# megvii-research/CVPR2023-UniDistill

Hardware: AMD Instinct MI355X
Metric: distill-train samples/sec (nuScenes frame); bev_pool+voxelize HBM GB/s (higher is better)
Workload: dtype f32; 1 GPU; camera_exp_distill_lidar: student+teacher distillation step, 6 cams 256x704, 30000-pt cloud, 40 GT boxes, fwd+bwd+AdamW; batch_per_gpu=4, global_batch=4, parallelism=dp1, layout=channels-last dense convs, executor=eager+DDP, strict_no_library_fallthrough=True, wgrad_stream=on, ranks=1, dist_backend=none (single process)

## Files before the change

### cvpr2023-unidistill_amd/csrc/bn_act.hip

```cpp
#include "ud_common.h"
#include "ud_prof.h"
#include "ud_reduce.h"

namespace {

constexpr int kMaxSlices = 1024;
int group_width(int C) { return C % 64 == 0 ? 64 : (C % 32 == 0 ? 32 : 16); }
int slices_for(long long P, int C) {
  const int gw = group_width(C), groups = C / gw;
  long long s = 2048 / (groups > 0 ? groups : 1);
  const long long cap = (P + 256 / (gw / 8) - 1) / (256 / (gw / 8));
  if (s > cap) s = cap;
  if (s < 1) s = 1;
  if (s > kMaxSlices) s = kMaxSlices;
  return (int)s;
}

__device__ __forceinline__ float bf_lo(unsigned u) { return __uint_as_float(u << 16); }
__device__ __forceinline__ float bf_hi(unsigned u) { return __uint_as_float(u & 0xFFFF0000u); }

__device__ __forceinline__ void unpack8(const uint4& r, float* v) {
  v[0] = bf_lo(r.x); v[1] = bf_hi(r.x); v[2] = bf_lo(r.y); v[3] = bf_hi(r.y);
  v[4] = bf_lo(r.z); v[5] = bf_hi(r.z); v[6] = bf_lo(r.w); v[7] = bf_hi(r.w);
}
__device__ __forceinline__ uint4 pack8(const float* v) {
  return make_uint4(ud_pack_bf16x2(v[0], v[1]), ud_pack_bf16x2(v[2], v[3]),
                    ud_pack_bf16x2(v[4], v[5]), ud_pack_bf16x2(v[6], v[7]));
}
__device__ __forceinline__ void ld8(const unsigned short* p, float* v) { unpack8(*reinterpret_cast<const uint4*>(p), v); }
__device__ __forceinline__ void st8(unsigned short* p, const float* v) { *reinterpret_cast<uint4*>(p) = pack8(v); }
__device__ __forceinline__ void ld8(const float* p, float* v) {
  const float4 a = *reinterpret_cast<const float4*>(p), b = *reinterpret_cast<const float4*>(p + 4);
  v[0] = a.x; v[1] = a.y; v[2] = a.z; v[3] = a.w; v[4] = b.x; v[5] = b.y; v[6] = b.z; v[7] = b.w;
}
__device__ __forceinline__ void st8(float* p, const float* v) {
  *reinterpret_cast<float4*>(p) = make_float4(v[0], v[1], v[2], v[3]);
  *reinterpret_cast<float4*>(p + 4) = make_float4(v[4], v[5], v[6], v[7]);
}
__device__ __forceinline__ float elem_f(unsigned short u) { return __uint_as_float((unsigned)u << 16); }
__device__ __forceinline__ float elem_f(float u) { return u; }

__device__ __forceinline__ void load8(const float* p, float* v) {
  const float4 a = *reinterpret_cast<const float4*>(p), b = *reinterpret_cast<const float4*>(p + 4);
  v[0] = a.x; v[1] = a.y; v[2] = a.z; v[3] = a.w; v[4] = b.x; v[5] = b.y; v[6] = b.z; v[7] = b.w;
}

template <typename T>
__global__ __launch_bounds__(256) void k_bn_act_fwd(const T* __restrict__ x, const T* __restrict__ res,
                                                    const float* __restrict__ scale,
                                                    const float* __restrict__ shift, T* __restrict__ y,
                                                    long long P, int C, int CH, int relu, long long y_ld) {
  const int chunk = blockIdx.y * CH + threadIdx.x % CH, lanes = 256 / CH, pl = threadIdx.x / CH;
  if (chunk * 8 >= C) return;
  float s[8], t[8];
  load8(scale + chunk * 8, s);
  load8(shift + chunk * 8, t);
  for (long long p = (long long)blockIdx.x * lanes + pl; p < P; p += (long long)gridDim.x * lanes) {
    const size_t off = (size_t)p * C + chunk * 8;
    float v[8];
    ld8(x + off, v);
#pragma unroll
    for (int e = 0; e < 8; ++e) v[e] = fmaf(v[e], s[e], t[e]);
    if (res) {
      float r[8];
      ld8(res + off, r);
#pragma unroll
      for (int e = 0; e < 8; ++e) v[e] += r[e];
    }
    if (relu) {
#pragma unroll
      for (int e = 0; e < 8; ++e) v[e] = fmaxf(v[e], 0.f);
    }
    st8(y + (size_t)p * y_ld + chunk * 8, v);
  }
}

__device__ __forceinline__ void masked_grad(const float* xv, const float* yv, bool has_y, const float* dyv,
                                            const float* s, const float* t, int relu, float* dr) {
  if (!relu) {
#pragma unroll
    for (int e = 0; e < 8; ++e) dr[e] = dyv[e];
    return;
  }
  if (has_y) {
#pragma unroll
    for (int e = 0; e < 8; ++e) dr[e] = yv[e] > 0.f ? dyv[e] : 0.f;
  } else {
#pragma unroll
    for (int e = 0; e < 8; ++e) dr[e] = fmaf(xv[e], s[e], t[e]) > 0.f ? dyv[e] : 0.f;
  }
}

template <int GW>
struct GroupMap {
  static constexpr int kChunks = GW / 8, kLanes = 256 / kChunks;
};

template <int GW, typename T>
__global__ __launch_bounds__(256) void k_bn_stats_partial(const T* __restrict__ x, long long P,
                                                          int C, float* __restrict__ partial) {
  using M = GroupMap<GW>;
  __shared__ float red[M::kLanes][GW + 1][2];
  const int cg = blockIdx.y, tid = threadIdx.x, chunk = tid % M::kChunks, pl = tid / M::kChunks;
  const int c0 = cg * GW + chunk * 8;
  float piv[8], s1[8], s2[8];
  ld8(x + c0, piv);
#pragma unroll
  for (int e = 0; e < 8; ++e) s1[e] = s2[e] = 0.f;
  for (long long p = (long long)blockIdx.x * M::kLanes + pl; p < P; p += (long long)gridDim.x * M::kLanes) {
    float v[8];
    ld8(x + (size_t)p * C + c0, v);
#pragma unroll
    for (int e = 0; e < 8; ++e) {
      const float d = v[e] - piv[e];
      s1[e] += d;
      s2[e] += d * d;
    }
  }
#pragma unroll
  for (int e = 0; e < 8; ++e) { red[pl][chunk * 8 + e][0] = s1[e]; red[pl][chunk * 8 + e][1] = s2[e]; }
  __syncthreads();
  if (tid < 2 * GW) {
    const int c = tid >> 1, w = tid & 1;
    float a = 0.f;
    for (int i = 0; i < M::kLanes; ++i) a += red[i][c][w];
    partial[((size_t)blockIdx.x * C + cg * GW + c) * 2 + w] = a;
  }
}

template <typename T>
__global__ __launch_bounds__(256) void k_bn_stats_final(const T* __restrict__ x, const float* __restrict__ partial,
                                 int slices, long long P, int C, const float* __restrict__ gamma,
                                 const float* __restrict__ beta, float eps, float* __restrict__ mean,
                                 float* __restrict__ var, float* __restrict__ invstd,
                                 float* __restrict__ scale, float* __restrict__ shift,
                                 float* __restrict__ running_mean, float* __restrict__ running_var,
                                 float momentum, long long* __restrict__ batches_tracked) {
  __shared__ double red[16][16][2];
  const int tid = threadIdx.x, cl = tid & 15, sl = tid >> 4;
  const int c = blockIdx.x * 16 + cl;
  if (batches_tracked && blockIdx.x == 0 && tid == 0) *batches_tracked += 1;
  auto ld = [&](int s) { return *reinterpret_cast<const float2*>(partial + ((size_t)s * C + c) * 2); };
  double a0 = 0.0, a1 = 0.0, a2 = 0.0, a3 = 0.0, q0 = 0.0, q1 = 0.0, q2 = 0.0, q3 = 0.0;
  int s = sl;
  for (; s + 48 < slices; s += 64) {
    const float2 v0 = ld(s), v1 = ld(s + 16), v2 = ld(s + 32), v3 = ld(s + 48);
    a0 += v0.x; q0 += v0.y;
    a1 += v1.x; q1 += v1.y;
    a2 += v2.x; q2 += v2.y;
    a3 += v3.x; q3 += v3.y;
  }
  for (; s < slices; s += 16) {
    const float2 v = ld(s);
    a0 += v.x; q0 += v.y;
  }
  double a = (a0 + a1) + (a2 + a3), q = (q0 + q1) + (q2 + q3);
  red[sl][cl][0] = a;
  red[sl][cl][1] = q;
  __syncthreads();
  if (sl != 0) return;
  a = q = 0.0;
  for (int k = 0; k < 16; ++k) {
    a += red[k][cl][0];
    q += red[k][cl][1];
  }
  const double piv = x ? (double)elem_f(x[c]) : 0.0;
  const double m = a / (double)P;
  double v = q / (double)P - m * m;
  if (v < 0.0) v = 0.0;
  const float mu = (float)(piv + m), is = (float)(1.0 / sqrt(v + (double)eps));
  mean[c] = mu;
  var[c] = (float)v;
  invstd[c] = is;
  const float sc = gamma[c] * is;
  scale[c] = sc;
  shift[c] = beta[c] - mu * sc;
  if (running_mean) {
    const double unbiased = v * ((double)P / (double)(P > 1 ? P - 1 : 1));
    running_mean[c] = (1.f - momentum) * running_mean[c] + momentum * mu;
    running_var[c] = (1.f - momentum) * running_var[c] + momentum * (float)unbiased;
  }
}

template <int GW, typename T>
__global__ __launch_bounds__(256) void k_bn_bwd_reduce(const T* __restrict__ x, const T* __restrict__ y,
                                                       const T* __restrict__ dy,
                                                       const float* __restrict__ scale,
                                                       const float* __restrict__ shift,
                                                       const float* __restrict__ mean, long long P,
                                                       int C, int relu, float* __restrict__ partial, long long dy_ld) {
  using M = GroupMap<GW>;
  __shared__ float red[M::kLanes][GW + 1][2];
  const int cg = blockIdx.y, tid = threadIdx.x, chunk = tid % M::kChunks, pl = tid / M::kChunks;
  const int c0 = cg * GW + chunk * 8;
  float s[8], t[8], mu[8], s1[8], s2[8];
  load8(scale + c0, s);
  load8(shift + c0, t);
  load8(mean + c0, mu);
#pragma unroll
  for (int e = 0; e < 8; ++e) s1[e] = s2[e] = 0.f;
  for (long long p = (long long)blockIdx.x * M::kLanes + pl; p < P; p += (long long)gridDim.x * M::kLanes) {
    const size_t off = (size_t)p * C + c0;
    float xv[8], dyv[8], dr[8], yv[8];
    ld8(x + off, xv);
    ld8(dy + (size_t)p * dy_ld + c0, dyv);
    if (y) ld8(y + off, yv);
    masked_grad(xv, yv, y != nullptr, dyv, s, t, relu, dr);
#pragma unroll
    for (int e = 0; e < 8; ++e) {
      s1[e] += dr[e];
      s2[e] += dr[e] * (xv[e] - mu[e]);
    }
  }
// ... 168 lines not shown
      a1 += elem_f(xp[(size_t)(p + step) * ld]);
    }
    if (p < P) a0 += elem_f(xp[(size_t)p * ld]);
  }
  red[tid] = a0 + a1;
  __syncthreads();
  if (tid < cw) {
    float a = 0.f;
    for (int i = 0; i < R; ++i) a += red[i * cw + tid];
    partial[(size_t)blockIdx.x * C + cb0 + tid] = a;
  }
}

struct BnWs { float *partial, *k0, *k2; };
size_t carve(UdArena& ar, int C, BnWs* w) {
  w->partial = ar.take<float>((size_t)kMaxSlices * C * 2);
  w->k0 = ar.take<float>(C);
  w->k2 = ar.take<float>(C);
  return ar.used;
}
void stream_grid(long long P, int C, int* CH, dim3* grid) {
  const int chunks = C / 8;
  int ch = 1;
  while (ch < chunks && ch < 256) ch <<= 1;
  const int lanes = 256 / ch, cblocks = (chunks + ch - 1) / ch;
  long long slices = (P + lanes - 1) / lanes;
  const long long want = 4096 / cblocks > 0 ? 4096 / cblocks : 1;
  if (slices > want) slices = want;
  if (slices < 1) slices = 1;
  *CH = ch;
  *grid = dim3((unsigned)slices, (unsigned)cblocks);
}

}

template <typename T>
int bn_stats_impl(const T* x, long long P, int C, const float* gamma, const float* beta, float eps,
                  float* mean, float* var, float* invstd, float* scale, float* shift, float* running_mean,
                  float* running_var, float momentum, long long* batches_tracked, void* workspace,
                  size_t workspace_bytes, hipStream_t stream) {
  if (!x || !gamma || !beta || !mean || !var || !invstd || !scale || !shift || P <= 0 || C <= 0 ||
      ((running_mean == nullptr) != (running_var == nullptr)))
    return UD_ERR_INVALID_ARG;
  if (C % 16) return UD_ERR_UNSUPPORTED;
  UdArena ar(workspace, workspace_bytes);
  BnWs w;
  carve(ar, C, &w);
  if (!ar.ok()) return UD_ERR_WORKSPACE;
  UdProfScope prof("bn_act.stats", stream);
  const int slices = slices_for(P, C), gw = group_width(C);
  if (gw == 64)
    k_bn_stats_partial<64, T><<<dim3(slices, C / 64), 256, 0, stream>>>(x, P, C, w.partial);
  else if (gw == 32)
    k_bn_stats_partial<32, T><<<dim3(slices, C / 32), 256, 0, stream>>>(x, P, C, w.partial);
  else
    k_bn_stats_partial<16, T><<<dim3(slices, C / 16), 256, 0, stream>>>(x, P, C, w.partial);
  UD_LAUNCH_CHECK();
  k_bn_stats_final<T><<<C / 16, 256, 0, stream>>>(x, w.partial, slices, P, C, gamma, beta, eps, mean, var, invstd, scale,
                                            shift, running_mean, running_var, momentum, batches_tracked);
  UD_LAUNCH_CHECK();
  return UD_OK;
}

template <typename T>
int bn_fwd_impl(const T* x, const T* residual, const float* scale, const float* shift, T* y, long long P, int C,
                int relu, long long y_ld, hipStream_t stream) {
// ... 140 lines not shown
                              float* shift, float* running_mean, float* running_var, float momentum,
                              long long* batches_tracked, ud_stream_t stream) {
  if (!partial || slices <= 0 || !gamma || !beta || !mean || !var || !invstd || !scale || !shift || P <= 0 || C <= 0 ||
      ((running_mean == nullptr) != (running_var == nullptr)))
    return UD_ERR_INVALID_ARG;
  UdProfScope prof("bn_act.stats", (hipStream_t)stream);
  if (C % 16) return UD_ERR_UNSUPPORTED;
  k_bn_stats_final<float><<<C / 16, 256, 0, (hipStream_t)stream>>>(nullptr, partial, slices, P, C, gamma, beta, eps, mean, var,
                                                              invstd, scale, shift, running_mean, running_var, momentum,
                                                              batches_tracked);
  UD_LAUNCH_CHECK();
  return UD_OK;
}

int ud_bn_act_fwd(const void* x, const void* residual, const float* scale, const float* shift, void* y,
                  long long P, int C, int relu, ud_stream_t stream) {
  return bn_fwd_impl<bf16_t>((const bf16_t*)x, (const bf16_t*)residual, scale, shift, (bf16_t*)y, P, C, relu, C,
                             (hipStream_t)stream);
}
int ud_bn_act_fwd_f32(const float* x, const float* residual, const float* scale, const float* shift, float* y,
                      long long P, int C, int relu, ud_stream_t stream) {
  return bn_fwd_impl<float>(x, residual, scale, shift, y, P, C, relu, C, (hipStream_t)stream);
}
int ud_bn_act_fwd_ld(const void* x, const void* residual, const float* scale, const float* shift, void* y,
                     long long P, int C, long long y_ld, int relu, ud_stream_t stream) {
  return bn_fwd_impl<bf16_t>((const bf16_t*)x, (const bf16_t*)residual, scale, shift, (bf16_t*)y, P, C, relu, y_ld,
                             (hipStream_t)stream);
}
int ud_bn_act_fwd_ld_f32(const float* x, const float* residual, const float* scale, const float* shift, float* y,
                         long long P, int C, long long y_ld, int relu, ud_stream_t stream) {
  return bn_fwd_impl<float>(x, residual, scale, shift, y, P, C, relu, y_ld, (hipStream_t)stream);
}

int ud_bn_act_bwd(const void* x, const void* y, const void* dy, const float* scale, const float* shift,
                  const float* mean, const float* invstd, void* dx, void* dresidual, float* dgamma,
                  float* dbeta, long long P, int C, int relu, void* workspace, size_t workspace_bytes,
                  ud_stream_t stream) {
  return bn_bwd_impl<bf16_t>((const bf16_t*)x, (const bf16_t*)y, (const bf16_t*)dy, scale, shift, mean, invstd,
                             (bf16_t*)dx, (bf16_t*)dresidual, dgamma, dbeta, P, C, relu, C, workspace, workspace_bytes,
                             (hipStream_t)stream);
}
int ud_bn_act_bwd_f32(const float* x, const float* y, const float* dy, const float* scale, const float* shift,
                      const float* mean, const float* invstd, float* dx, float* dresidual, float* dgamma,
                      float* dbeta, long long P, int C, int relu, void* workspace, size_t workspace_bytes,
                      ud_stream_t stream) {
  return bn_bwd_impl<float>(x, y, dy, scale, shift, mean, invstd, dx, dresidual, dgamma, dbeta, P, C, relu, C, workspace,
                            workspace_bytes, (hipStream_t)stream);
}
int ud_bn_act_bwd_ld(const void* x, const void* y, const void* dy, long long dy_ld, const float* scale, const float* shift,
                     const float* mean, const float* invstd, void* dx, void* dresidual, float* dgamma,
                     float* dbeta, long long P, int C, int relu, void* workspace, size_t workspace_bytes,
                     ud_stream_t stream) {
  return bn_bwd_impl<bf16_t>((const bf16_t*)x, (const bf16_t*)y, (const bf16_t*)dy, scale, shift, mean, invstd,
                             (bf16_t*)dx, (bf16_t*)dresidual, dgamma, dbeta, P, C, relu, dy_ld, workspace, workspace_bytes,
                             (hipStream_t)stream);
}
int ud_bn_act_bwd_ld_f32(const float* x, const float* y, const float* dy, long long dy_ld, const float* scale,
                         const float* shift, const float* mean, const float* invstd, float* dx, float* dresidual,
                         float* dgamma, float* dbeta, long long P, int C, int relu, void* workspace,
                         size_t workspace_bytes, ud_stream_t stream) {
  return bn_bwd_impl<float>(x, y, dy, scale, shift, mean, invstd, dx, dresidual, dgamma, dbeta, P, C, relu, dy_ld,
                            workspace, workspace_bytes, (hipStream_t)stream);
}
int ud_bn_act_bwd_frozen_ld(const void* x, const void* y, const void* dy, long long dy_ld, const float* scale,
                            const float* shift, const float* mean, const float* invstd, void* dx, void* dresidual,
                            float* dgamma, float* dbeta, long long P, int C, int relu, void* workspace,
// ... 25 lines not shown
```

### cvpr2023-unidistill_amd/csrc/ud_reduce.h

```cpp
#ifndef UD_REDUCE_H_
#define UD_REDUCE_H_
#include "ud_common.h"

namespace {

__global__ __launch_bounds__(256) void k_wgrad_sum(const float* __restrict__ partial, int slices, size_t n,
                                                   float* __restrict__ out) {
  __shared__ float4 part[4][64];
  const int lane = threadIdx.x & 63, wave = threadIdx.x >> 6;
  const size_t i4 = (size_t)blockIdx.x * 64 + lane, n4 = n / 4;
  float4 a = make_float4(0.f, 0.f, 0.f, 0.f);
  if (i4 < n4) {
    const int per = (slices + 3) / 4, s0 = wave * per, s1 = min(slices, s0 + per);
    auto ld = [&](int s) { return *reinterpret_cast<const float4*>(partial + (size_t)s * n + 4 * i4); };
    int s = s0;
    for (; s + 3 < s1; s += 4) {
      const float4 v0 = ld(s), v1 = ld(s + 1), v2 = ld(s + 2), v3 = ld(s + 3);
      a.x += v0.x; a.y += v0.y; a.z += v0.z; a.w += v0.w;
      a.x += v1.x; a.y += v1.y; a.z += v1.z; a.w += v1.w;
      a.x += v2.x; a.y += v2.y; a.z += v2.z; a.w += v2.w;
      a.x += v3.x; a.y += v3.y; a.z += v3.z; a.w += v3.w;
    }
    for (; s < s1; ++s) {
      const float4 v = ld(s);
// ... 57 lines not shown
#pragma unroll
  for (int o = 32; o > 0; o >>= 1) {
    a += __shfl_xor(a, o);
    q += __shfl_xor(q, o);
  }
  if (T > 64) {
    if (lane == 0) { red[wv][0] = a; red[wv][1] = q; }
    __syncthreads();
    if (tid == 0) {
      a = red[0][0], q = red[0][1];
#pragma unroll
      for (int w = 1; w < T / 64; ++w) { a += red[w][0]; q += red[w][1]; }
    }
  }
  if (tid != 0) return;
  const float is = invstd[c], dg = q * is, inv_p = 1.0f / (float)P;
  dbeta[c] = a;
  dgamma[c] = dg;
  const float kk2 = -scale[c] * (dg * inv_p) * is;
  k2[c] = kk2;
  k0[c] = -scale[c] * (a * inv_p) - kk2 * mean[c];
}

inline int ud_bn_bwd_final(const float* partial, int slices, int C, long long P, const float* scale, const float* mean,
                           const float* invstd, float* dgamma, float* dbeta, float* k0, float* k2, hipStream_t stream) {
  if (slices > 128)
    k_bn_bwd_final<256><<<C, 256, 0, stream>>>(partial, slices, C, P, scale, mean, invstd, dgamma, dbeta, k0, k2);
  else
    k_bn_bwd_final<64><<<C, 64, 0, stream>>>(partial, slices, C, P, scale, mean, invstd, dgamma, dbeta, k0, k2);
  UD_LAUNCH_CHECK();
  return UD_OK;
}

template <int T, typename V>
__device__ __forceinline__ V ud_colsum_block(const V* __restrict__ partial, int slices, int C, int c, V* __restrict__ red) {
  const int tid = threadIdx.x, lane = tid & 63, wv = tid >> 6;
  V a0 = 0, a1 = 0, a2 = 0, a3 = 0;
  int s = tid;
  for (; s + 3 * T < slices; s += 4 * T) {
    const V v0 = partial[(size_t)s * C + c], v1 = partial[(size_t)(s + T) * C + c], v2 = partial[(size_t)(s + 2 * T) * C + c],
            v3 = partial[(size_t)(s + 3 * T) * C + c];
    a0 += v0; a1 += v1; a2 += v2; a3 += v3;
  }
  for (; s < slices; s += T) a0 += partial[(size_t)s * C + c];
  V a = (a0 + a1) + (a2 + a3);
#pragma unroll
  for (int o = 32; o > 0; o >>= 1) a += __shfl_xor(a, o);
  if (T > 64) {
    if (lane == 0) red[wv] = a;
    __syncthreads();
    if (tid == 0) {
      a = red[0];
#pragma unroll
      for (int w = 1; w < T / 64; ++w) a += red[w];
    }
  }
  return a;
}

template <int T>
__global__ __launch_bounds__(T) void k_colsum_final(const float* __restrict__ partial, int slices, int C, float* __restrict__ out) {
  __shared__ float red[T / 64];
  const float a = ud_colsum_block<T, float>(partial, slices, C, blockIdx.x, red);
  if (threadIdx.x == 0) out[blockIdx.x] = a;
}

// ... 56 lines not shown
```

### cvpr2023-unidistill_amd/unidistill_amd/ops/bn_act.py

```python
import torch

from .. import _lib


def supported(x, bn):
    if not (x.is_cuda and x.dtype in (torch.bfloat16, torch.float32) and x.dim() in (2, 4) and x.shape[1] % 16 == 0
            and x.shape[0] > 0 and bn.affine and bn.track_running_stats and bn.momentum is not None):
        return False
    return x.is_contiguous() if x.dim() == 2 else x.is_contiguous(memory_format=torch.channels_last)


def _like(t, ref):
    t = t.to(ref.dtype)
    return t.contiguous() if ref.dim() == 2 else t.contiguous(memory_format=torch.channels_last)


def _row_stride(t, ref):
    if t.dim() != 4 or ref.dim() != 4 or t.dtype != ref.dtype or t.shape != ref.shape or not t.is_cuda:
        return None
    B, C, H, W = t.shape
    s = t.stride()
    ld = s[3] if W > 1 else (s[2] if H > 1 else C)
    if ld < C or ld % 8 or t.data_ptr() % 16 or (C > 1 and s[1] != 1) or (W > 1 and s[3] != ld) or (H > 1 and s[2] != W * ld) \
            or (B > 1 and s[0] != H * W * ld):
        return None
    return ld


_ws_bytes = {}


def _workspace(dev, C):
    n = _ws_bytes.get(C)
    if n is None:
        n = _ws_bytes[C] = _lib.load().ud_bn_act_workspace_bytes(C)
    return _lib.workspace(dev, n, "bn_act")


def batch_stats(x, gamma, beta, running_mean, running_var, training, momentum, eps, tracked=None, partial=None):
    _lib.require_gpu(x, gamma, beta)
    f32 = x.dtype == torch.float32
    k_stats = _lib.ud.ud_bn_stats_f32 if f32 else _lib.ud.ud_bn_stats
    C = x.shape[1]
    P = x.numel() // C
    dev = x.device
    g32 = gamma.detach() if gamma.dtype == torch.float32 else gamma.detach().float()
    b32 = beta.detach() if beta.dtype == torch.float32 else beta.detach().float()
    stream = _lib.stream_of(x)
    if training:
        vec = torch.empty((5, C), dtype=torch.float32, device=dev)
        v0, row = vec.data_ptr(), 4 * C
        ws = _workspace(dev, C)
        fp32_buffers = running_mean is not None and running_mean.dtype == torch.float32
        rm, rv = (running_mean, running_var) if fp32_buffers else (None, None)
        if partial is not None and partial[2] == P:
            _lib.ud.ud_bn_stats_from_partials(partial[0].data_ptr(), int(partial[1]), P, C, g32.data_ptr(), b32.data_ptr(),
                                              float(eps), v0, v0 + row, v0 + 2 * row, v0 + 3 * row, v0 + 4 * row, rm, rv,
                                              float(momentum or 0.0), tracked, stream)
        else:
            k_stats(x.data_ptr(), P, C, g32.data_ptr(), b32.data_ptr(), float(eps), v0, v0 + row, v0 + 2 * row, v0 + 3 * row,
                    v0 + 4 * row, rm, rv, float(momentum or 0.0), tracked, ws.data_ptr(), ws.numel(), stream)
        if rm is not None:
            torch.autograd.graph.increment_version(rm)
            torch.autograd.graph.increment_version(rv)
        if running_mean is not None and not fp32_buffers:
            with torch.no_grad():
                running_mean.mul_(1 - momentum).add_(vec[0], alpha=momentum)
                running_var.mul_(1 - momentum).add_(vec[1], alpha=momentum * P / max(P - 1, 1))
        return vec
    def fold():
        invstd = torch.rsqrt(running_var.float() + eps)
        mean = running_mean.float()
        scale = g32 * invstd
        return torch.stack((mean, invstd * invstd, invstd, scale, b32 - mean * scale))

    if gamma.requires_grad or beta.requires_grad or torch.cuda.is_current_stream_capturing():
        if getattr(running_var, "_ud_bn_eval", None) is not None and not torch.cuda.is_current_stream_capturing():
            running_var._ud_bn_eval = None
        return fold()
    key = (running_mean._version, running_var._version, gamma._version, beta._version, float(eps),
           running_mean.data_ptr(), running_var.data_ptr(), gamma.data_ptr(), beta.data_ptr())
    hit = getattr(running_var, "_ud_bn_eval", None)
    if hit is not None and hit[0] == key:
        return hit[1]
    vec = fold()
    try:
        running_var._ud_bn_eval = (key, vec)
    except (AttributeError, RuntimeError):
# ... 10 lines not shown


def drop_colsum(g):
    if getattr(g, "_ud_colsum", None) is not None:
        g._ud_colsum = None


def bias_grad(gy):
    hit = getattr(gy, "_ud_colsum", None)
    if hit is not None and hit[0] == gy._version and hit[1] == gy.data_ptr():
        return hit[2]
    C = gy.shape[1]
    rows = gy.dim() == 2 and gy.is_contiguous()
    maps = gy.dim() == 4 and gy.is_contiguous(memory_format=torch.channels_last)
    if not (gy.is_cuda and gy.dtype in (torch.float32, torch.bfloat16) and (rows or maps) and gy.numel() > 0):
        dims = (0,) if gy.dim() == 2 else (0, 2, 3)
        return gy.sum(dims, dtype=torch.float32)
    lib = _lib.load()
    out = torch.empty(C, dtype=torch.float32, device=gy.device)
    ws = _lib.workspace(gy.device, lib.ud_colsum_workspace_bytes(C), "colsum")
    fn = _lib.ud.ud_colsum_f32 if gy.dtype == torch.float32 else _lib.ud.ud_colsum_bf16
    fn(gy.data_ptr(), gy.numel() // C, C, C, out.data_ptr(), ws.data_ptr(), ws.numel(), _lib.stream_of(gy))
    return out


class _BnActFn(torch.autograd.Function):
    @staticmethod
    def forward(ctx, x, gamma, beta, residual, running_mean, running_var, training, momentum, eps, relu,
                tracked=None, partial=None, out=None):
        k_fwd = _lib.ud.ud_bn_act_fwd_ld_f32 if x.dtype == torch.float32 else _lib.ud.ud_bn_act_fwd_ld
        C = x.shape[1]
        P = x.numel() // C
        stream = _lib.stream_of(x)
        vec = batch_stats(x, gamma, beta, running_mean, running_var, training, momentum, eps, tracked, partial)
        v0, row = vec.data_ptr(), 4 * C
        if residual is not None:
            residual = _like(residual, x)
        y = torch.empty_like(x) if out is None else out[0]
        ld = C if out is None else _row_stride(y, x)
        if ld is None:
            raise ValueError(f"bn_act: out {tuple(y.shape)} strides {tuple(y.stride())} is not a channel slice of a channels-last map")
        k_fwd(x.data_ptr(), residual, v0 + 3 * row, v0 + 4 * row, y.data_ptr(), P, C, ld, 1 if relu else 0, stream)
        ctx.cfg = (bool(training), bool(relu), residual is not None)
        ctx.save_for_backward(x, y if (residual is not None and relu) else None, vec)
        return y

    @staticmethod
    def backward(ctx, dy):
        x, y, vec = ctx.saved_tensors
        training, relu, has_res = ctx.cfg
        if y is not None and y.stride() != x.stride():
            y = _like(y, x)
        C = x.shape[1]
        P = x.numel() // C
        ld = _row_stride(dy, x)
        if ld is None:
            dy, ld = _like(dy, x), C
        dx = torch.empty_like(x)
        dres = torch.empty_like(x) if (has_res and ctx.needs_input_grad[3]) else None
        if dres is not None and not relu:
            dres = None
        v0, row = vec.data_ptr(), 4 * C
        if training:
            dgb = torch.empty((2, C), dtype=torch.float32, device=x.device)
            ws = _workspace(x.device, C)
            g0 = dgb.data_ptr()
            k_bwd = _lib.ud.ud_bn_act_bwd_ld_f32 if x.dtype == torch.float32 else _lib.ud.ud_bn_act_bwd_ld
            k_bwd(x.data_ptr(), y, dy.data_ptr(), ld, v0 + 3 * row, v0 + 4 * row, v0, v0 + 2 * row, dx.data_ptr(), dres, g0,
                  g0 + row, P, C, 1 if relu else 0, ws.data_ptr(), ws.numel(), _lib.stream_of(x))
            dgamma, dbeta = dgb[0], dgb[1]
        else:
            k_bwd = _lib.ud.ud_bn_act_bwd_frozen_ld_f32 if x.dtype == torch.float32 else _lib.ud.ud_bn_act_bwd_frozen_ld
            dgamma = dbeta = dgb = ws = None
            if ctx.needs_input_grad[1] or ctx.needs_input_grad[2]:
                dgb = torch.empty((2, C), dtype=torch.float32, device=x.device)
# ... 64 lines not shown
```

### include/unidistill_hip.h

```cpp
#ifndef UNIDISTILL_HIP_H
#define UNIDISTILL_HIP_H

#include <stddef.h>
#include <stdint.h>

#ifdef __cplusplus
extern "C" {
#endif

typedef void* ud_stream_t;

#define UD_OK 0
#define UD_ERR_INVALID_ARG (-1)
#define UD_ERR_WORKSPACE (-2)
#define UD_ERR_HIP (-3)
#define UD_ERR_UNSUPPORTED (-4)

const char* ud_version(void);
int ud_abi_version(void);
const char* ud_error_string(int code);

void ud_prof_enable(int on);
int ud_prof_read(const char* name, double* total_ms, int* calls, int reset);

// ... 373 lines not shown
size_t ud_bn_act_workspace_bytes(int C);
int ud_bn_stats(const void* x, long long P, int C, const float* gamma, const float* beta, float eps,
                float* mean, float* var, float* invstd, float* scale, float* shift, float* running_mean,
                float* running_var, float momentum, long long* batches_tracked, void* workspace,
                size_t workspace_bytes, ud_stream_t stream);
int ud_bn_act_fwd(const void* x, const void* residual, const float* scale, const float* shift, void* y,
                  long long P, int C, int relu, ud_stream_t stream);
int ud_bn_act_bwd(const void* x, const void* y, const void* dy, const float* scale, const float* shift,
                  const float* mean, const float* invstd, void* dx, void* dresidual, float* dgamma,
                  float* dbeta, long long P, int C, int relu, void* workspace, size_t workspace_bytes,
                  ud_stream_t stream);
int ud_bn_stats_from_partials(const float* partial, int slices, long long P, int C, const float* gamma,
                              const float* beta, float eps, float* mean, float* var, float* invstd, float* scale,
                              float* shift, float* running_mean, float* running_var, float momentum,
                              long long* batches_tracked, ud_stream_t stream);
int ud_bn_stats_f32(const float* x, long long P, int C, const float* gamma, const float* beta, float eps,
                    float* mean, float* var, float* invstd, float* scale, float* shift, float* running_mean,
                    float* running_var, float momentum, long long* batches_tracked, void* workspace,
                    size_t workspace_bytes, ud_stream_t stream);
int ud_bn_act_fwd_f32(const float* x, const float* residual, const float* scale, const float* shift, float* y,
                      long long P, int C, int relu, ud_stream_t stream);
int ud_bn_act_bwd_f32(const float* x, const float* y, const float* dy, const float* scale, const float* shift,
                      const float* mean, const float* invstd, float* dx, float* dresidual, float* dgamma,
                      float* dbeta, long long P, int C, int relu, void* workspace, size_t workspace_bytes,
                      ud_stream_t stream);
int ud_bn_act_fwd_ld(const void* x, const void* residual, const float* scale, const float* shift, void* y,
                     long long P, int C, long long y_ld, int relu, ud_stream_t stream);
int ud_bn_act_fwd_ld_f32(const float* x, const float* residual, const float* scale, const float* shift, float* y,
                         long long P, int C, long long y_ld, int relu, ud_stream_t stream);
int ud_bn_act_bwd_ld(const void* x, const void* y, const void* dy, long long dy_ld, const float* scale, const float* shift,
                     const float* mean, const float* invstd, void* dx, void* dresidual, float* dgamma,
                     float* dbeta, long long P, int C, int relu, void* workspace, size_t workspace_bytes,
                     ud_stream_t stream);
int ud_bn_act_bwd_ld_f32(const float* x, const float* y, const float* dy, long long dy_ld, const float* scale,
                         const float* shift, const float* mean, const float* invstd, float* dx, float* dresidual,
                         float* dgamma, float* dbeta, long long P, int C, int relu, void* workspace,
                         size_t workspace_bytes, ud_stream_t stream);
int ud_bn_act_bwd_frozen_ld(const void* x, const void* y, const void* dy, long long dy_ld, const float* scale,
                            const float* shift, const float* mean, const float* invstd, void* dx, void* dresidual,
                            float* dgamma, float* dbeta, long long P, int C, int relu, void* workspace,
                            size_t workspace_bytes, ud_stream_t stream);
int ud_bn_act_bwd_frozen_ld_f32(const float* x, const float* y, const float* dy, long long dy_ld, const float* scale,
                                const float* shift, const float* mean, const float* invstd, float* dx, float* dresidual,
                                float* dgamma, float* dbeta, long long P, int C, int relu, void* workspace,
                                size_t workspace_bytes, ud_stream_t stream);

size_t ud_nms_bev_workspace_bytes(int N);
int ud_nms_rotated_bev(const float* boxes, int N, float thresh, long long* keep, int* num_keep,
                       void* workspace, size_t workspace_bytes, ud_stream_t stream);
int ud_boxes_iou_bev(const float* a, int Na, const float* b, int Nb, float* iou, ud_stream_t stream);

size_t ud_proposal_workspace_bytes(int B, int T, int K);
int ud_proposal_layer(const float* const* heads, const long long* strides, const int* num_classes,
                      const int* class_offsets, const float* iou_alpha, int B, int T, int H, int W, int K,
                      int post_max, int box_dim, int no_log, float out_size_factor, float voxel_x,
                      float voxel_y, float pc_x, float pc_y, const float* center_range, float score_threshold,
                      float nms_threshold, float* rois, float* roi_scores, long long* roi_labels,
                      int* num_boxes, void* workspace, size_t workspace_bytes, ud_stream_t stream);

size_t ud_det_loss_workspace_bytes(int T);
int ud_det_focal_fwd(const float* const* hm, const long long* hm_bstride, const int* ncls, int T, int B,
                     int ncm, int HW, const float* gt, float alpha, float gamma, float* prob,
                     float* pos_neg, void* workspace, size_t workspace_bytes, ud_stream_t stream);
int ud_det_focal_bwd(const int* ncls, int T, int B, int ncm, int HW, const float* gt, const float* prob,
                     const float* g_prob, const float* g_pos, const float* g_neg, float alpha,
                     float gamma, float* dlogit, ud_stream_t stream);
// ... 284 lines not shown
```

Before: 70.06 samples/s.

## Fold BN stats finalization into the training forward apply kernel

Adds a training-mode BN forward path in which each apply block reduces the per-slice partial sums for its channel group, computes scale/shift in shared memory, and then applies BN+residual+ReLU. This removes the separate k_bn_stats_final launch and the global round-trip of scale/shift. The apply loop is also unrolled 4x to keep more loads in flight. In exchange, every block redundantly re-reduces the partials (only block 0 writes the stats), and the fold is limited to at most 64 slices, falling back to the old path otherwise.

```diff
diff --git a/cvpr2023-unidistill_amd/csrc/bn_act.hip b/cvpr2023-unidistill_amd/csrc/bn_act.hip
--- a/cvpr2023-unidistill_amd/csrc/bn_act.hip
+++ b/cvpr2023-unidistill_amd/csrc/bn_act.hip
@@ -43,6 +43,19 @@
 __device__ __forceinline__ void load8(const float* p, float* v) {
   const float4 a = *reinterpret_cast<const float4*>(p), b = *reinterpret_cast<const float4*>(p + 4);
   v[0] = a.x; v[1] = a.y; v[2] = a.z; v[3] = a.w; v[4] = b.x; v[5] = b.y; v[6] = b.z; v[7] = b.w;
+}
+
+__device__ __forceinline__ void bn_apply8(float* v, const float* r, bool has_r, const float* s, const float* t, int relu) {
+#pragma unroll
+  for (int e = 0; e < 8; ++e) v[e] = fmaf(v[e], s[e], t[e]);
+  if (has_r) {
+#pragma unroll
+    for (int e = 0; e < 8; ++e) v[e] += r[e];
+  }
+  if (relu) {
+#pragma unroll
+    for (int e = 0; e < 8; ++e) v[e] = fmaxf(v[e], 0.f);
+  }
 }
 
 template <typename T>
@@ -57,20 +70,10 @@
   load8(shift + chunk * 8, t);
   for (long long p = (long long)blockIdx.x * lanes + pl; p < P; p += (long long)gridDim.x * lanes) {
     const size_t off = (size_t)p * C + chunk * 8;
-    float v[8];
+    float v[8], r[8];
     ld8(x + off, v);
-#pragma unroll
-    for (int e = 0; e < 8; ++e) v[e] = fmaf(v[e], s[e], t[e]);
-    if (res) {
-      float r[8];
-      ld8(res + off, r);
-#pragma unroll
-      for (int e = 0; e < 8; ++e) v[e] += r[e];
-    }
-    if (relu) {
-#pragma unroll
-      for (int e = 0; e < 8; ++e) v[e] = fmaxf(v[e], 0.f);
-    }
+    if (res) ld8(res + off, r);
+    bn_apply8(v, r, res != nullptr, s, t, relu);
     st8(y + (size_t)p * y_ld + chunk * 8, v);
   }
 }
@@ -125,6 +128,21 @@
     float a = 0.f;
     for (int i = 0; i < M::kLanes; ++i) a += red[i][c][w];
     partial[((size_t)blockIdx.x * C + cg * GW + c) * 2 + w] = a;
+  }
+}
+
+__device__ __forceinline__ void bn_store_stats(const UdBnFwdStats& st, int c, float* __restrict__ mean, float* __restrict__ var,
+                                               float* __restrict__ invstd, float* __restrict__ scale, float* __restrict__ shift,
+                                               float* __restrict__ running_mean, float* __restrict__ running_var,
+                                               float momentum) {
+  mean[c] = st.mean;
+  var[c] = st.var;
+  invstd[c] = st.invstd;
+  scale[c] = st.scale;
+  shift[c] = st.shift;
+  if (running_mean) {
+    running_mean[c] = (1.f - momentum) * running_mean[c] + momentum * st.mean;
+    running_var[c] = (1.f - momentum) * running_var[c] + momentum * st.unbiased;
   }
 }
 
@@ -140,21 +158,8 @@
   const int tid = threadIdx.x, cl = tid & 15, sl = tid >> 4;
   const int c = blockIdx.x * 16 + cl;
   if (batches_tracked && blockIdx.x == 0 && tid == 0) *batches_tracked += 1;
-  auto ld = [&](int s) { return *reinterpret_cast<const float2*>(partial + ((size_t)s * C + c) * 2); };
-  double a0 = 0.0, a1 = 0.0, a2 = 0.0, a3 = 0.0, q0 = 0.0, q1 = 0.0, q2 = 0.0, q3 = 0.0;
-  int s = sl;
-  for (; s + 48 < slices; s += 64) {
-    const float2 v0 = ld(s), v1 = ld(s + 16), v2 = ld(s + 32), v3 = ld(s + 48);
-    a0 += v0.x; q0 += v0.y;
-    a1 += v1.x; q1 += v1.y;
-    a2 += v2.x; q2 += v2.y;
-    a3 += v3.x; q3 += v3.y;
-  }
-  for (; s < slices; s += 16) {
-    const float2 v = ld(s);
-    a0 += v.x; q0 += v.y;
-  }
-  double a = (a0 + a1) + (a2 + a3), q = (q0 + q1) + (q2 + q3);
+  double a, q;
+  ud_bn_fwd_lane_sums<1>(partial, slices, C, &c, &sl, &a, &q);
   red[sl][cl][0] = a;
   red[sl][cl][1] = q;
   __syncthreads();
@@ -164,21 +169,84 @@
     a += red[k][cl][0];
     q += red[k][cl][1];
   }
-  const double piv = x ? (double)elem_f(x[c]) : 0.0;
-  const double m = a / (double)P;
-  double v = q / (double)P - m * m;
-  if (v < 0.0) v = 0.0;
-  const float mu = (float)(piv + m), is = (float)(1.0 / sqrt(v + (double)eps));
-  mean[c] = mu;
-  var[c] = (float)v;
-  invstd[c] = is;
-  const float sc = gamma[c] * is;
-  scale[c] = sc;
-  shift[c] = beta[c] - mu * sc;
-  if (running_mean) {
-    const double unbiased = v * ((double)P / (double)(P > 1 ? P - 1 : 1));
-    running_mean[c] = (1.f - momentum) * running_mean[c] + momentum * mu;
-    running_var[c] = (1.f - momentum) * running_var[c] + momentum * (float)unbiased;
+  const UdBnFwdStats st = ud_bn_fwd_channel(a, q, x ? (double)elem_f(x[c]) : 0.0, P, gamma[c], beta[c], eps);
+  bn_store_stats(st, c, mean, var, invstd, scale, shift, running_mean, running_var, momentum);
+}
+
+template <typename T>
+__global__ __launch_bounds__(256) void k_bn_act_fwd_fold(const T* __restrict__ x, const T* __restrict__ res,
+                                                         const float* __restrict__ partial, int slices, int pivot,
+                                                         const float* __restrict__ gamma, const float* __restrict__ beta,
+                                                         float eps, float* __restrict__ mean, float* __restrict__ var,
+                                                         float* __restrict__ invstd, float* __restrict__ scale,
+                                                         float* __restrict__ shift, float* __restrict__ running_mean,
+                                                         float* __restrict__ running_var, float momentum,
+                                                         long long* __restrict__ batches_tracked, T* __restrict__ y,
+                                                         long long P, int C, int CH, int relu, long long y_ld) {
+  __shared__ double red[16][64][2];
+  __shared__ float s_scale[64], s_shift[64];
+  const int tid = threadIdx.x, cb0 = blockIdx.y * CH * 8, nch = min(CH * 8, C - cb0);
+  if (batches_tracked && blockIdx.x == 0 && blockIdx.y == 0 && tid == 0) *batches_tracked += 1;
+  {
+    int c[4], sl[4];
+    double a[4], q[4];
+#pragma unroll
+    for (int k = 0; k < 4; ++k) {
+      const int i = min(tid + 256 * k, nch * 16 - 1);
+      sl[k] = i / nch;
+      c[k] = cb0 + i % nch;
+    }
+    ud_bn_fwd_lane_sums<4>(partial, slices, C, c, sl, a, q);
+#pragma unroll
+    for (int k = 0; k < 4; ++k)
+      if (tid + 256 * k < nch * 16) {
+        red[sl[k]][c[k] - cb0][0] = a[k];
+        red[sl[k]][c[k] - cb0][1] = q[k];
+      }
+  }
+  __syncthreads();
+  if (tid < nch) {
+    const int c = cb0 + tid;
+    double a = 0.0, q = 0.0;
+    for (int k = 0; k < 16; ++k) {
+      a += red[k][tid][0];
+      q += red[k][tid][1];
+    }
+    const UdBnFwdStats st = ud_bn_fwd_channel(a, q, pivot ? (double)elem_f(x[c]) : 0.0, P, gamma[c], beta[c], eps);
+    s_scale[tid] = st.scale;
+    s_shift[tid] = st.shift;
+    if (blockIdx.x == 0) bn_store_stats(st, c, mean, var, invstd, scale, shift, running_mean, running_var, momentum);
+  }
+  __syncthreads();
+  const int ck = tid % CH, lanes = 256 / CH, pl = tid / CH;
+  if (ck * 8 >= nch) return;
+  const int c0 = cb0 + ck * 8;
+  float s[8], t[8];
+#pragma unroll
+  for (int e = 0; e < 8; ++e) { s[e] = s_scale[ck * 8 + e]; t[e] = s_shift[ck * 8 + e]; }
+  const long long step = (long long)gridDim.x * lanes;
+  long long p = (long long)blockIdx.x * lanes + pl;
+  for (; p + 3 * step < P; p += 4 * step) {
+    float v[4][8], r[4][8];
+#pragma unroll
+    for (int u = 0; u < 4; ++u) {
+      const size_t off = (size_t)(p + u * step) * C + c0;
+      ld8(x + off, v[u]);
+      if (res) ld8(res + off, r[u]);
+    }
+#pragma unroll
+    for (int u = 0; u < 4; ++u) {
+      bn_apply8(v[u], r[u], res != nullptr, s, t, relu);
+      st8(y + (size_t)(p + u * step) * y_ld + c0, v[u]);
+    }
+  }
+  for (; p < P; p += step) {
+    const size_t off = (size_t)p * C + c0;
+    float v[8], r[8];
+    ld8(x + off, v);
+    if (res) ld8(res + off, r);
+    bn_apply8(v, r, res != nullptr, s, t, relu);
+    st8(y + (size_t)p * y_ld + c0, v);
   }
 }
 
@@ -413,6 +481,74 @@
   *grid = dim3((unsigned)slices, (unsigned)cblocks);
 }
 
+constexpr int kFoldMaxSlices = 64;
+bool fold_plan(long long P, int C, int slices, int* CH, dim3* grid) {
+  if (C % 16 || slices < 1 || slices > kFoldMaxSlices) return false;
+  const int chunks = C / 8;
+  int ch = 1;
+  while (ch < chunks && ch < 8) ch <<= 1;
+  const int lanes = 256 / ch, cblocks = (chunks + ch - 1) / ch;
+  const long long rows = (P + lanes - 1) / lanes, want = 2048 / cblocks > 0 ? 2048 / cblocks : 1, cap = P / (2ll * slices);
+  long long s = rows < want ? rows : want;
+  if (s > cap) s = cap;
+  if (s < 1 || (s < rows && s * cblocks < 256) || cblocks > 65535) return false;
+  *CH = ch;
+  *grid = dim3((unsigned)s, (unsigned)cblocks);
+  return true;
+}
+
+}
+
+template <typename T>
+int bn_fwd_impl(const T* x, const T* residual, const float* scale, const float* shift, T* y, long long P, int C,
+                int relu, long long y_ld, hipStream_t stream);
+
+template <typename T>
+int bn_train_fwd_impl(const T* x, const T* residual, const float* partial, int slices, const float* gamma, const float* beta,
+                      float eps, float* mean, float* var, float* invstd, float* scale, float* shift, float* running_mean,
+                      float* running_var, float momentum, long long* batches_tracked, T* y, long long P, int C, int relu,
+                      long long y_ld, void* workspace, size_t workspace_bytes, hipStream_t stream) {
+  if (!x || !gamma || !beta || !mean || !var || !invstd || !scale || !shift || !y || P <= 0 || C <= 0 || y_ld < C ||
+      ((running_mean == nullptr) != (running_var == nullptr)) || (partial && slices <= 0))
+    return UD_ERR_INVALID_ARG;
+  if (C % 16 || y_ld % 8 || ((size_t)y & 15)) return UD_ERR_UNSUPPORTED;
+  const bool own = partial == nullptr;
+  BnWs w;
+  if (own) {
+    UdArena ar(workspace, workspace_bytes);
+    carve(ar, C, &w);
+    if (!ar.ok()) return UD_ERR_WORKSPACE;
+    slices = slices_for(P, C);
+    partial = w.partial;
+  }
+  int CH;
+  dim3 grid;
+  const bool fold = fold_plan(P, C, slices, &CH, &grid);
+  if (own || !fold) {
+    UdProfScope prof("bn_act.stats", stream);
+    if (own) {
+      const int gw = group_width(C);
+      if (gw == 64)
+        k_bn_stats_partial<64, T><<<dim3(slices, C / 64), 256, 0, stream>>>(x, P, C, w.partial);
+      else if (gw == 32)
+        k_bn_stats_partial<32, T><<<dim3(slices, C / 32), 256, 0, stream>>>(x, P, C, w.partial);
+      else
+        k_bn_stats_partial<16, T><<<dim3(slices, C / 16), 256, 0, stream>>>(x, P, C, w.partial);
+      UD_LAUNCH_CHECK();
+    }
+    if (!fold) {
+      k_bn_stats_final<T><<<C / 16, 256, 0, stream>>>(own ? x : nullptr, partial, slices, P, C, gamma, beta, eps, mean, var,
+                                                      invstd, scale, shift, running_mean, running_var, momentum, batches_tracked);
+      UD_LAUNCH_CHECK();
+    }
+  }
+  if (!fold) return bn_fwd_impl<T>(x, residual, scale, shift, y, P, C, relu, y_ld, stream);
+  UdProfScope prof("bn_act.k_fwd", stream);
+  k_bn_act_fwd_fold<T><<<grid, 256, 0, stream>>>(x, residual, partial, slices, own ? 1 : 0, gamma, beta, eps, mean, var, invstd,
+                                                 scale, shift, running_mean, running_var, momentum, batches_tracked, y, P, C, CH,
+                                                 relu, y_ld);
+  UD_LAUNCH_CHECK();
+  return UD_OK;
 }
 
 template <typename T>
@@ -619,6 +755,31 @@
   return bn_fwd_impl<float>(x, residual, scale, shift, y, P, C, relu, y_ld, (hipStream_t)stream);
 }
 
+int ud_bn_act_train_fwd_ld(const void* x, const void* residual, const float* partial, int slices, const float* gamma,
+                           const float* beta, float eps, float* mean, float* var, float* invstd, float* scale, float* shift,
+                           float* running_mean, float* running_var, float momentum, long long* batches_tracked, void* y,
+                           long long P, int C, long long y_ld, int relu, void* workspace, size_t workspace_bytes,
+                           ud_stream_t stream) {
+  return bn_train_fwd_impl<bf16_t>((const bf16_t*)x, (const bf16_t*)residual, partial, slices, gamma, beta, eps, mean, var,
+                                   invstd, scale, shift, running_mean, running_var, momentum, batches_tracked, (bf16_t*)y, P, C,
+                                   relu, y_ld, workspace, workspace_bytes, (hipStream_t)stream);
+}
+int ud_bn_act_train_fwd_ld_f32(const float* x, const float* residual, const float* partial, int slices, const float* gamma,
+                               const float* beta, float eps, float* mean, float* var, float* invstd, float* scale, float* shift,
+                               float* running_mean, float* running_var, float momentum, long long* batches_tracked, float* y,
+                               long long P, int C, long long y_ld, int relu, void* workspace, size_t workspace_bytes,
+                               ud_stream_t stream) {
+  return bn_train_fwd_impl<float>(x, residual, partial, slices, gamma, beta, eps, mean, var, invstd, scale, shift, running_mean,
+                                  running_var, momentum, batches_tracked, y, P, C, relu, y_ld, workspace, workspace_bytes,
+                                  (hipStream_t)stream);
+}
+int ud_bn_act_train_fwd_folds(long long P, int C, int slices) {
+  if (P <= 0 || C <= 0 || C % 16) return 0;
+  int CH;
+  dim3 grid;
+  return fold_plan(P, C, slices > 0 ? slices : slices_for(P, C), &CH, &grid) ? 1 : 0;
+}
+
 int ud_bn_act_bwd(const void* x, const void* y, const void* dy, const float* scale, const float* shift,
                   const float* mean, const float* invstd, void* dx, void* dresidual, float* dgamma,
                   float* dbeta, long long P, int C, int relu, void* workspace, size_t workspace_bytes,
diff --git a/cvpr2023-unidistill_amd/csrc/ud_reduce.h b/cvpr2023-unidistill_amd/csrc/ud_reduce.h
--- a/cvpr2023-unidistill_amd/csrc/ud_reduce.h
+++ b/cvpr2023-unidistill_amd/csrc/ud_reduce.h
@@ -113,6 +113,61 @@
   return UD_OK;
 }
 
+template <int K>
+__device__ __forceinline__ void ud_bn_fwd_lane_sums(const float* __restrict__ partial, int slices, int C, const int* c, const int* sl,
+                                                    double* a, double* q) {
+  double acc[K][4], sq[K][4];
+#pragma unroll
+  for (int k = 0; k < K; ++k)
+#pragma unroll
+    for (int j = 0; j < 4; ++j) acc[k][j] = sq[k][j] = 0.0;
+  auto ld = [&](int k, int s) { return *reinterpret_cast<const float2*>(partial + ((size_t)s * C + c[k]) * 2); };
+  for (int s0 = 0; s0 < slices; s0 += 64) {
+    float2 v[K][4];
+    bool ok[K][4];
+#pragma unroll
+    for (int k = 0; k < K; ++k) {
+      const int s = s0 + sl[k];
+      const bool full = s + 48 < slices;
+#pragma unroll
+      for (int j = 0; j < 4; ++j) {
+        ok[k][j] = s + 16 * j < slices;
+        v[k][j] = ok[k][j] ? ld(k, s + 16 * j) : make_float2(0.f, 0.f);
+      }
+      if (full) {
+#pragma unroll
+        for (int j = 0; j < 4; ++j) { acc[k][j] += v[k][j].x; sq[k][j] += v[k][j].y; }
+      } else {
+#pragma unroll
+        for (int j = 0; j < 4; ++j)
+          if (ok[k][j]) { acc[k][0] += v[k][j].x; sq[k][0] += v[k][j].y; }
+      }
+    }
+  }
+#pragma unroll
+  for (int k = 0; k < K; ++k) {
+    a[k] = (acc[k][0] + acc[k][1]) + (acc[k][2] + acc[k][3]);
+    q[k] = (sq[k][0] + sq[k][1]) + (sq[k][2] + sq[k][3]);
+  }
+}
+
+struct UdBnFwdStats { float mean, var, invstd, scale, shift, unbiased; };
+
+__device__ __forceinline__ UdBnFwdStats ud_bn_fwd_channel(double a, double q, double piv, long long P, float gamma, float beta,
+                                                          float eps) {
+  const double m = a / (double)P;
+  double v = q / (double)P - m * m;
+  if (v < 0.0) v = 0.0;
+  UdBnFwdStats o;
+  o.mean = (float)(piv + m);
+  o.invstd = (float)(1.0 / sqrt(v + (double)eps));
+  o.var = (float)v;
+  o.scale = gamma * o.invstd;
+  o.shift = beta - o.mean * o.scale;
+  o.unbiased = (float)(v * ((double)P / (double)(P > 1 ? P - 1 : 1)));
+  return o;
+}
+
 template <int T, typename V>
 __device__ __forceinline__ V ud_colsum_block(const V* __restrict__ partial, int slices, int C, int c, V* __restrict__ red) {
   const int tid = threadIdx.x, lane = tid & 63, wv = tid >> 6;
diff --git a/cvpr2023-unidistill_amd/unidistill_amd/ops/bn_act.py b/cvpr2023-unidistill_amd/unidistill_amd/ops/bn_act.py
--- a/cvpr2023-unidistill_amd/unidistill_amd/ops/bn_act.py
+++ b/cvpr2023-unidistill_amd/unidistill_amd/ops/bn_act.py
@@ -37,7 +37,7 @@
     return _lib.workspace(dev, n, "bn_act")
 
 
-def batch_stats(x, gamma, beta, running_mean, running_var, training, momentum, eps, tracked=None, partial=None):
+def batch_stats(x, gamma, beta, running_mean, running_var, training, momentum, eps, tracked=None, partial=None, apply=None):
     _lib.require_gpu(x, gamma, beta)
     f32 = x.dtype == torch.float32
     k_stats = _lib.ud.ud_bn_stats_f32 if f32 else _lib.ud.ud_bn_stats
@@ -53,7 +53,14 @@
         ws = _workspace(dev, C)
         fp32_buffers = running_mean is not None and running_mean.dtype == torch.float32
         rm, rv = (running_mean, running_var) if fp32_buffers else (None, None)
-        if partial is not None and partial[2] == P:
+        from_conv = partial is not None and partial[2] == P
+        if apply is not None:
+            residual, y, ld, relu = apply
+            k_train = _lib.ud.ud_bn_act_train_fwd_ld_f32 if f32 else _lib.ud.ud_bn_act_train_fwd_ld
+            k_train(x.data_ptr(), residual, partial[0].data_ptr() if from_conv else None, int(partial[1]) if from_conv else 0,
+                    g32.data_ptr(), b32.data_ptr(), float(eps), v0, v0 + row, v0 + 2 * row, v0 + 3 * row, v0 + 4 * row, rm, rv,
+                    float(momentum or 0.0), tracked, y.data_ptr(), P, C, ld, 1 if relu else 0, ws.data_ptr(), ws.numel(), stream)
+        elif from_conv:
             _lib.ud.ud_bn_stats_from_partials(partial[0].data_ptr(), int(partial[1]), P, C, g32.data_ptr(), b32.data_ptr(),
                                               float(eps), v0, v0 + row, v0 + 2 * row, v0 + 3 * row, v0 + 4 * row, rm, rv,
                                               float(momentum or 0.0), tracked, stream)
@@ -130,15 +137,19 @@
         C = x.shape[1]
         P = x.numel() // C
         stream = _lib.stream_of(x)
-        vec = batch_stats(x, gamma, beta, running_mean, running_var, training, momentum, eps, tracked, partial)
-        v0, row = vec.data_ptr(), 4 * C
         if residual is not None:
             residual = _like(residual, x)
         y = torch.empty_like(x) if out is None else out[0]
         ld = C if out is None else _row_stride(y, x)
         if ld is None:
             raise ValueError(f"bn_act: out {tuple(y.shape)} strides {tuple(y.stride())} is not a channel slice of a channels-last map")
-        k_fwd(x.data_ptr(), residual, v0 + 3 * row, v0 + 4 * row, y.data_ptr(), P, C, ld, 1 if relu else 0, stream)
+        if training:
+            vec = batch_stats(x, gamma, beta, running_mean, running_var, True, momentum, eps, tracked, partial,
+                              apply=(residual, y, ld, relu))
+        else:
+            vec = batch_stats(x, gamma, beta, running_mean, running_var, False, momentum, eps)
+            v0, row = vec.data_ptr(), 4 * C
+            k_fwd(x.data_ptr(), residual, v0 + 3 * row, v0 + 4 * row, y.data_ptr(), P, C, ld, 1 if relu else 0, stream)
         ctx.cfg = (bool(training), bool(relu), residual is not None)
         ctx.save_for_backward(x, y if (residual is not None and relu) else None, vec)
         return y
diff --git a/include/unidistill_hip.h b/include/unidistill_hip.h
--- a/include/unidistill_hip.h
+++ b/include/unidistill_hip.h
@@ -429,6 +429,17 @@
                      const float* mean, const float* invstd, void* dx, void* dresidual, float* dgamma,
                      float* dbeta, long long P, int C, int relu, void* workspace, size_t workspace_bytes,
                      ud_stream_t stream);
+int ud_bn_act_train_fwd_ld(const void* x, const void* residual, const float* partial, int slices, const float* gamma,
+                           const float* beta, float eps, float* mean, float* var, float* invstd, float* scale, float* shift,
+                           float* running_mean, float* running_var, float momentum, long long* batches_tracked, void* y,
+                           long long P, int C, long long y_ld, int relu, void* workspace, size_t workspace_bytes,
+                           ud_stream_t stream);
+int ud_bn_act_train_fwd_ld_f32(const float* x, const float* residual, const float* partial, int slices, const float* gamma,
+                               const float* beta, float eps, float* mean, float* var, float* invstd, float* scale, float* shift,
+                               float* running_mean, float* running_var, float momentum, long long* batches_tracked, float* y,
+                               long long P, int C, long long y_ld, int relu, void* workspace, size_t workspace_bytes,
+                               ud_stream_t stream);
+int ud_bn_act_train_fwd_folds(long long P, int C, int slices);
 int ud_bn_act_bwd_ld_f32(const float* x, const float* y, const float* dy, long long dy_ld, const float* scale,
                          const float* shift, const float* mean, const float* invstd, float* dx, float* dresidual,
                          float* dgamma, float* dbeta, long long P, int C, int relu, void* workspace,
```

Measured after the change: 69.73 samples/s. Within noise of the previous version (-0.5%).
